# hbell99/DirectVoxGO

Hardware: AMD Instinct MI355X
Metric: train rays/sec (8192-ray batch, 160^3 grid) (higher is better)
Workload: dtype f32

## Files before the change

### directvoxgo_amd/_lib.py

```python
import ctypes
import os
import re

import torch

_HERE = os.path.dirname(os.path.abspath(__file__))
SO_PATH = os.environ.get('DVGO_HIP_SO') or os.path.join(_HERE, 'csrc', 'libdvgo_hip.so')
ABI_VERSION = 11
HEADER_PATH = os.path.join(os.path.dirname(_HERE), 'include', 'dvgo_hip.h')

_lib = None
_nargs = {}


class _Rec2(ctypes.Structure):
    _fields_ = [('step', ctypes.c_int32), ('exp_d', ctypes.c_float), ('alpha', ctypes.c_float), ('T', ctypes.c_float)]


_vp = ctypes.c_void_p
_i64 = ctypes.c_int64
_int = ctypes.c_int
_flt = ctypes.c_float


# ... 87 lines not shown


class _NoCtx:
    def __enter__(self):
        return self

    def __exit__(self, *exc):
        return False


_NOCTX = _NoCtx()


def device_of(t):
    if t.device.index == torch.cuda.current_device():
        return _NOCTX
    return torch.cuda.device_of(t)


_ERR = {-1: 'invalid argument', -2: 'size exceeds 32-bit launch range'}


_profile = None


def profile_start(names):
    global _profile
    _profile = {n: [] for n in names}


def profile_stop():
    global _profile
    prof, _profile = _profile, None
    torch.cuda.synchronize()
    return {n: (len(ev), sum(a.elapsed_time(b) for a, b in ev)) for n, ev in (prof or {}).items()}


def call(name, *args):
    handle = lib()
    if len(args) != _nargs.get(name):
        raise TypeError(f'{name}: {len(args)} arguments given, include/dvgo_hip.h declares {_nargs.get(name, "no such function")}')
    fn = getattr(handle, name)
    if _profile is not None and name in _profile:
        a, b = torch.cuda.Event(enable_timing=True), torch.cuda.Event(enable_timing=True)
        a.record()
        rc = fn(*args)
        b.record()
        _profile[name].append((a, b))
    else:
        rc = fn(*args)
    if rc != 0:
        raise RuntimeError(f'{name} failed: {_ERR.get(rc, "hipError %d" % rc)}')


def f3(x):
    if isinstance(x, torch.Tensor):
        x = x.detach().cpu().tolist()
    return (ctypes.c_float * 3)(*[float(v) for v in x])
```

### directvoxgo_amd/csrc/shade.hip

```cpp
#include "common.h"
#include "x3.h"

#include <type_traits>


static int g_shade_experiment = 0;
static int g_shade_variant = 67;
extern "C" int dvgo_shade_wgrad_x3(const float* G1, const float* gz, const uint64_t* masks, const float* W3, const float* H1,
                                   const float* H2, const float* feat, int C, const float* emb, int E, const int64_t* ray_id,
                                   int64_t M, const int64_t* m_dev, int width, int diffuse, int n_parts, float* part, int form_b,
                                   void* stream);
extern "C" int dvgo_shade_bwd_x3(const float* g_rgb, const float* rgb, const uint64_t* masks, int64_t M, const int64_t* m_dev,
                                 const float* W1, const float* W2, const float* W3, int width, int d_in, int C, int diffuse,
                                 float* g_feat, float* G1, float* gz, void* scratch, int prebuilt, void* stream);

extern "C" int dvgo_shade_fwd_x3(const float* feat, int C, const float* emb, int E, const int64_t* ray_id, int64_t M, const int64_t* m_dev,
                                 const float* W1, const float* b1, const float* W2, const float* b2, const float* W3,
                                 const float* b3, int width, int d_in, int diffuse, float* rgb, float* H1, float* H2,
                                 uint64_t* masks, void* scratch, void* scratch_bwd, int experiment, void* stream);

#define SHADE_THREADS 768
#define SHADE_WAVES (SHADE_THREADS / 64)
#define SHADE_BWD_THREADS 1024
#define SHADE_BWD_WAVES (SHADE_BWD_THREADS / 64)
// ... 977 lines not shown
#pragma unroll
  for (int r = 0; r < 16; ++r) {
    const int i = (r & 3) + 8 * (r >> 2) + 4 * h;
#pragma unroll
    for (int t = 0; t < T; ++t) pW2[(32 * w + i) * WIDTH + 32 * t + j] = aW2[t][r];
    pW1[(32 * w + i) * 64 + j] = aW1[0][r];
    pW1[(32 * w + i) * 64 + 32 + j] = aW1[1][r];
  }
#pragma unroll
  for (int c = 0; c < 3; ++c) {
    const float v = vW3[c] + __shfl_xor(vW3[c], 32);
    if (h == 0) pW3[c * WIDTH + 32 * w + j] = v;
    sgz[c] += __shfl_xor(sgz[c], 32);
  }
  sb1 += __shfl_xor(sb1, 32); sb2 += __shfl_xor(sb2, 32);
  if (h == 0) {
    pb[32 * w + j] = sb1;
    pb[WIDTH + 32 * w + j] = sb2;
    if (j < 8) pb[2 * WIDTH + 8 * w + j] = (w == 0 && j < 3) ? sgz[j] : 0.0f;
    if (T == 2 && j >= 16) pb[2 * WIDTH + 16 * w + j] = 0.0f;
  }
#endif
}
#undef DVGO_OOB

#define SHADE_REDUCE_SLICES 16
__global__ void __launch_bounds__(256)
shade_wgrad_reduce_kernel(const float* __restrict__ part, int n_parts, int n, int W, int d_in, float* __restrict__ out) {
  const int i = blockIdx.x * blockDim.x + threadIdx.x;
  if (i >= n) return;
  int o;
  const int nW2 = W * W, nW1 = W * 64, nW3 = 32 * W;
  if (i < nW2) o = i;
  else if (i < nW2 + nW1) {
    const int r = (i - nW2) >> 6, c = (i - nW2) & 63;
    o = c < d_in ? nW2 + r * d_in + c : -1;
  } else if (i < nW2 + nW1 + nW3) {
    const int e = i - nW2 - nW1;
    o = e < 3 * W ? nW2 + W * d_in + e : -1;
  } else {
    const int e = i - nW2 - nW1 - nW3, base = nW2 + W * d_in + 3 * W;
    if (e < 2 * W) o = base + e;
    else {
      const int c = e - 2 * W;
      o = c < 3 ? base + 2 * W + c : (c >= 8 && c < 11) ? base + 2 * W + c - 8 : -1;
    }
// ... 2 lines not shown
  const int per = (n_parts + SHADE_REDUCE_SLICES - 1) / SHADE_REDUCE_SLICES;
  const int p0 = blockIdx.y * per, p1 = min(n_parts, p0 + per);
  float a0 = 0.0f, a1 = 0.0f, a2 = 0.0f, a3 = 0.0f;
  int p = p0;
  for (; p + 4 <= p1; p += 4) {
    a0 += part[(int64_t)p * n + i];
    a1 += part[(int64_t)(p + 1) * n + i];
    a2 += part[(int64_t)(p + 2) * n + i];
    a3 += part[(int64_t)(p + 3) * n + i];
  }
  for (; p < p1; ++p) a0 += part[(int64_t)p * n + i];
  if (p1 > p0) atomicAdd(out + o, (a0 + a1) + (a2 + a3));
}

extern "C" {

int dvgo_shade_fwd(const float* feat, int C, const float* emb, int E, const int64_t* ray_id, int64_t M, const int64_t* m_dev,
                   const float* W1, const float* b1, const float* W2, const float* b2, const float* W3,
                   const float* b3, int width, int d_in, int diffuse, float* rgb, float* H1, float* H2,
                   uint64_t* masks, void* scratch, void* scratch_bwd, void* stream) {
  if (M < 0 || C <= 0 || E < 0) return DVGO_EINVAL;
  if (M == 0) return 0;
  if (!feat || !emb || !ray_id || !W1 || !b1 || !W2 || !b2 || !W3 || !b3 || !rgb) return DVGO_EINVAL;
  if ((H1 == nullptr) != (H2 == nullptr) || (H1 == nullptr) != (masks == nullptr)) return DVGO_EINVAL;
  const int c_view0 = diffuse ? 3 : 0;
  const int n_view = C - c_view0;
  if (n_view < 0 || d_in != n_view + E) return DVGO_EINVAL;
  if ((width != 128 && width != 64) || d_in > 40) return DVGO_ERANGE;
  if ((g_shade_variant & 1) && scratch != nullptr)
    return dvgo_shade_fwd_x3(feat, C, emb, E, ray_id, M, m_dev, W1, b1, W2, b2, W3, b3, width, d_in, diffuse, rgb, H1, H2, masks,
                             scratch, (g_shade_variant & 2) ? scratch_bwd : nullptr, g_shade_experiment, stream);
  hipStream_t s = (hipStream_t)stream;
  const int64_t n_tiles = (M + 31) / 32;
  const int64_t cap = width == 128 ? 256 : 512;
  int blocks = (int)((n_tiles + SHADE_WAVES - 1) / SHADE_WAVES < cap ? (n_tiles + SHADE_WAVES - 1) / SHADE_WAVES : cap);
#define DVGO_SHADE(W, S1, DIFF)                                                                           \
  shade_fwd_kernel<W, S1, DIFF><<<blocks, SHADE_THREADS, 0, s>>>(feat, C, c_view0, n_view, emb, E, ray_id, M, m_dev, W1, b1, W2, \
                                                          b2, W3, b3, d_in, rgb, H1, H2, (unsigned long long*)masks, g_shade_experiment)
  if (width == 128) {
    if (d_in <= 36) { if (diffuse) DVGO_SHADE(128, 18, true); else DVGO_SHADE(128, 18, false); }
    else            { if (diffuse) DVGO_SHADE(128, 20, true); else DVGO_SHADE(128, 20, false); }
  } else {
    if (d_in <= 12) { if (diffuse) DVGO_SHADE(64, 6, true); else DVGO_SHADE(64, 6, false); }
    else            { if (diffuse) DVGO_SHADE(64, 20, true); else DVGO_SHADE(64, 20, false); }
  }
#undef DVGO_SHADE
  DVGO_LAUNCH_CHECK();
// ... 58 lines not shown
    else if (width == 128)
      shade_wgrad_ring_kernel<128><<<n_parts, 256, 0, (hipStream_t)stream>>>(
          G1, gz, (const unsigned int*)masks, W3, H1, H2, feat, C, c_view0, n_view, emb, E, ray_id, M, m_dev, part, total, tsz);
    else
      shade_wgrad_ring_kernel<64><<<n_parts, 128, 0, (hipStream_t)stream>>>(
          G1, gz, (const unsigned int*)masks, W3, H1, H2, feat, C, c_view0, n_view, emb, E, ray_id, M, m_dev, part, total, tsz);
  } else if (width == 128)
    shade_wgrad_kernel<128><<<n_parts, 256, 0, (hipStream_t)stream>>>(
        G1, gz, (const unsigned int*)masks, W3, H1, H2, feat, C, c_view0, n_view, emb, E, ray_id, M, m_dev, part);
  else
    shade_wgrad_kernel<64><<<n_parts, 128, 0, (hipStream_t)stream>>>(
        G1, gz, (const unsigned int*)masks, W3, H1, H2, feat, C, c_view0, n_view, emb, E, ray_id, M, m_dev, part);
  DVGO_LAUNCH_CHECK();
  const int psize = width * width + width * 64 + 32 * width + 3 * width;
  const int d_in = n_view + E;
  const int tsize = width * width + width * d_in + 3 * width + 2 * width + 3;
  if (!ring && hipMemsetAsync(total, 0, (size_t)tsize * sizeof(float), (hipStream_t)stream) != hipSuccess) return DVGO_EINVAL;
  shade_wgrad_reduce_kernel<<<dim3((psize + 255) / 256, SHADE_REDUCE_SLICES), 256, 0, (hipStream_t)stream>>>(part, n_parts, psize,
                                                                                                       width, d_in, total);
  DVGO_LAUNCH_CHECK();
  return 0;
}

}
```

### directvoxgo_amd/csrc/shade_x3.hip

```cpp
#include "common.h"
#include "x3.h"

#ifndef X3_THREADS
#define X3_THREADS 512
#endif
#define X3_WAVES (X3_THREADS / 64)
#ifndef X3_BWD_THREADS
#define X3_BWD_THREADS 512
#endif
#define X3_BWD_WAVES (X3_BWD_THREADS / 64)
#define X3_STAGE_ROWS 16
#define X3_STAGE_STRIDE 36

__device__ __forceinline__ int x3_acc_feature(int t, int r, int h) { return 32 * t + (r & 3) + 8 * (r >> 2) + 4 * h; }

__device__ __forceinline__ void x3_split1(float v, unsigned short& s0, unsigned short& s1, unsigned short& s2) {
  const unsigned int h = x3_pack(v, 0.f) & 0xffffu;
  const float r = v - __uint_as_float(h << 16);
  const unsigned int m = x3_pack(r, 0.f) & 0xffffu;
  const float q = r - __uint_as_float(m << 16);
  s0 = (unsigned short)h; s1 = (unsigned short)m; s2 = (unsigned short)(x3_pack(q, 0.f) & 0xffffu);
}

template <int WIDTH, int KS1>
// ... 75 lines not shown
  }
  for (int i = tid; i < 2 * T * 16; i += nt) {
    const int tr = i % (T * 16), h = i / (T * 16);
    const int f = x3_acc_feature(tr >> 4, tr & 15, h);
    (&L.b1p[0][0])[i] = b1[f];
    (&L.b2p[0][0])[i] = b2[f];
  }
  if (tid < 4) L.b3[tid] = tid < 3 ? b3[tid] : 0.0f;
}

template <int WIDTH, int KS1, bool DIFFUSE>
__global__ void __launch_bounds__(X3_THREADS)
shade_fwd_x3_kernel(const float* __restrict__ feat, int C, int c_view0, int n_view, const float* __restrict__ emb, int E,
                    const int64_t* __restrict__ ray_id, int64_t M_cap, const int64_t* __restrict__ m_dev,
                    const void* __restrict__ image, float* __restrict__ rgb,
                    float* __restrict__ H1, float* __restrict__ H2, unsigned long long* __restrict__ masks, int experiment) {
  const int64_t M = m_dev ? (*m_dev < M_cap ? *m_dev : M_cap) : M_cap;
  constexpr int T = WIDTH / 32;
  __shared__ __attribute__((aligned(16))) X3Lds<WIDTH, KS1> L;
  x3_copy_image<X3Img<WIDTH, KS1>>(&L, image);
  __syncthreads();
  const int lane = threadIdx.x & 63, h = lane >> 5;
  float* stage = L.stage[threadIdx.x >> 6];
  const bool train = H1 != nullptr;
  const int64_t n_tiles = (M + 31) / 32;
  const int64_t gw = (int64_t)blockIdx.x * (blockDim.x >> 6) + (threadIdx.x >> 6);
  const int64_t nw = (int64_t)gridDim.x * (blockDim.x >> 6);
  const int d_in = n_view + E;
  const int64_t last = M > 0 ? M - 1 : 0;
  auto row_of = [&](int64_t tile) { const int64_t r = tile * 32 + (lane & 31); return r < M ? r : last; };
  float xin[KS1][8];
  auto load_inputs = [&](int64_t tile, int64_t rid) {
    const float* fr = feat + row_of(tile) * C + c_view0;
    const float* er = emb + rid * E - n_view;
#pragma unroll
    for (int s = 0; s < KS1; ++s)
#pragma unroll
      for (int j = 0; j < 8; ++j) {
        const int k = 16 * s + 8 * h + j;
        const int kc = k < d_in ? k : d_in - 1;
        xin[s][j] = *((kc < n_view) ? fr + kc : er + kc);
      }
  };
  int64_t rid_n = 0;
  if (gw < n_tiles) { load_inputs(gw, ray_id[row_of(gw)]); rid_n = ray_id[row_of(gw + nw)]; }
  for (int64_t tile = gw; tile < n_tiles; tile += nw) {
    const int64_t row = tile * 32 + (lane & 31);
// ... 6 lines not shown
#pragma unroll
      for (int j = 0; j < 8; ++j) v[j] = (16 * s + 8 * h + j) < d_in ? xin[s][j] : 0.0f;
      x3_split8(v, x3[s][0], x3[s][1], x3[s][2]);
    }
    load_inputs(tile + nw, rid_n);
    rid_n = ray_id[row_of(tile + 2 * nw)];
    u32x4 h3[2 * T][3];
    unsigned long long mask1 = 0ull;
#pragma unroll
    for (int t = 0; t < T; ++t) {
      f32x16 acc;
#pragma unroll
      for (int r = 0; r < 16; ++r) acc[r] = L.b1p[h][t * 16 + r];
#pragma unroll
      for (int s = 0; s < KS1; ++s)
        x3_mfma6(acc, L.w1s[t][s][0][lane], L.w1s[t][s][1][lane], L.w1s[t][s][2][lane], x3[s][0], x3[s][1], x3[s][2]);
#pragma unroll
      for (int r = 0; r < 16; ++r) acc[r] = dvgo_relu(acc[r]);
      if (train) {
        unsigned int bits = 0u;
#pragma unroll
        for (int r = 0; r < 16; ++r) bits |= dvgo_relu_bit(acc[r]) << r;
        mask1 |= (unsigned long long)bits << (16 * t);
        if (!(experiment & 512)) x3_store_tile(stage, acc, H1 + tile * 32 * WIDTH + 32 * t, WIDTH, lane, rows_valid);
      }
#pragma unroll
      for (int s2 = 0; s2 < 2; ++s2) {
        float v[8];
#pragma unroll
        for (int j = 0; j < 8; ++j) v[j] = acc[8 * s2 + j];
        x3_split8(v, h3[2 * t + s2][0], h3[2 * t + s2][1], h3[2 * t + s2][2]);
      }
      __builtin_amdgcn_sched_barrier(0);
    }
    float p[3] = {0.0f, 0.0f, 0.0f};
    unsigned long long mask2 = 0ull;
#pragma unroll 1
    for (int t2 = 0; t2 < T; ++t2) {
      f32x16 acc2;
#pragma unroll
      for (int r = 0; r < 16; ++r) acc2[r] = L.b2p[h][t2 * 16 + r];
      u32x4 a[2][3];
#pragma unroll
      for (int q = 0; q < 3; ++q) a[0][q] = L.w2s[t2][0][q][lane];
#pragma unroll
      for (int ks = 0; ks < 2 * T; ++ks) {
        if (ks + 1 < 2 * T) {
// ... 892 lines not shown
      float s1 = sb1[t] + red[half][TA * 2 * 16 * 64 + 64 * t + lane];
      s1 += __shfl_xor(s1, 32);
      if (h == 0) pb[T * i + tile] = s1;
    }
  }
#endif
}

extern "C" {

int64_t dvgo_shade_scratch_bytes(int width) {
  if (width == 128) return (int64_t)sizeof(X3Img<128, 3>) > (int64_t)sizeof(X3BwdImg<128>) ? sizeof(X3Img<128, 3>) : sizeof(X3BwdImg<128>);
  if (width == 64) return (int64_t)sizeof(X3Img<64, 3>) > (int64_t)sizeof(X3BwdImg<64>) ? sizeof(X3Img<64, 3>) : sizeof(X3BwdImg<64>);
  return 0;
}

int dvgo_shade_fwd_x3(const float* feat, int C, const float* emb, int E, const int64_t* ray_id, int64_t M, const int64_t* m_dev,
                      const float* W1, const float* b1, const float* W2, const float* b2, const float* W3,
                      const float* b3, int width, int d_in, int diffuse, float* rgb, float* H1, float* H2,
                      uint64_t* masks, void* scratch, void* scratch_bwd, int experiment, void* stream) {
  if (M < 0 || C <= 0 || E < 0) return DVGO_EINVAL;
  if (M == 0) return 0;
  if (!feat || !emb || !ray_id || !W1 || !b1 || !W2 || !b2 || !W3 || !b3 || !rgb || !scratch) return DVGO_EINVAL;
  if ((H1 == nullptr) != (H2 == nullptr) || (H1 == nullptr) != (masks == nullptr)) return DVGO_EINVAL;
  const int c_view0 = diffuse ? 3 : 0;
  const int n_view = C - c_view0;
  if (n_view < 0 || d_in != n_view + E) return DVGO_EINVAL;
  if ((width != 128 && width != 64) || d_in > 48) return DVGO_ERANGE;
  hipStream_t s = (hipStream_t)stream;
  const int64_t n_tiles = (M + 31) / 32;
  const int64_t cap = 256;
  const int blocks = (int)((n_tiles + X3_WAVES - 1) / X3_WAVES < cap ? (n_tiles + X3_WAVES - 1) / X3_WAVES : cap);
#define DVGO_SHADE_X3(W, KS, DIFF)                                                                                       \
  do {                                                                                                                   \
    x3_prep_fwd_kernel<W, KS><<<scratch_bwd ? 64 : 32, 256, 0, s>>>((X3Img<W, KS>*)scratch, (X3BwdImg<W>*)scratch_bwd, W1, b1, W2, b2, W3, b3, d_in); \
    shade_fwd_x3_kernel<W, KS, DIFF><<<blocks, X3_THREADS, 0, s>>>(feat, C, c_view0, n_view, emb, E, ray_id, M, m_dev, scratch, rgb, \
                                                                    H1, H2, (unsigned long long*)masks, experiment);     \
  } while (0)
  if (width == 128) {
    if (diffuse) DVGO_SHADE_X3(128, 3, true); else DVGO_SHADE_X3(128, 3, false);
  } else {
    if (d_in <= 16) { if (diffuse) DVGO_SHADE_X3(64, 1, true); else DVGO_SHADE_X3(64, 1, false); }
    else            { if (diffuse) DVGO_SHADE_X3(64, 3, true); else DVGO_SHADE_X3(64, 3, false); }
  }
#undef DVGO_SHADE_X3
  DVGO_LAUNCH_CHECK();
  return 0;
// ... 63 lines not shown
```

### directvoxgo_amd/shade.py

```python

import torch
import torch.nn as nn

from . import _lib as L
from ._lib import _i64, _int, ptr, stream_of

N_PARTS = 512


class defer_wgrad:
    _active = None
    _streams = {}

    def __init__(self, side_stream=True):
        self.side_stream = side_stream

    def __enter__(self):
        self.pending = []
        defer_wgrad._active = self
        return self

    def __exit__(self, *exc):
        defer_wgrad._active = None
        return False
# ... 56 lines not shown
    gW3 = tot[o:o + 3 * width].view(3, width); o += 3 * width
    gb1, gb2, gb3 = tot[o:o + width], tot[o + width:o + 2 * width], tot[o + 2 * width:o + 2 * width + 3]
    return gW1, gb1, gW2, gb2, gW3, gb3


def _weight_grads(params, wgrad, device, k, n, g_first=None):
    grads = [g_first] + [None] * (n - 1)
    if defer_wgrad._active is not None:
        defer_wgrad._active.submit(params, wgrad, device)
    else:
        grads[k:k + 6] = wgrad()
    return tuple(grads)


class _Shade(torch.autograd.Function):
    @staticmethod
    def forward(ctx, feat, emb, ray_id, W1, b1, W2, b2, W3, b3, diffuse, train, m_dev):
        M, C = feat.shape
        E = emb.shape[1]
        width, d_in = W1.shape
        feat, emb = feat.contiguous(), emb.contiguous()
        train = bool(train) and any(ctx.needs_input_grad)
        rgb = torch.empty((M, 3), dtype=torch.float32, device=feat.device)
        H1 = torch.empty((M, width), dtype=torch.float32, device=feat.device) if train else None
        H2 = torch.empty((M, width), dtype=torch.float32, device=feat.device) if train else None
        masks = torch.empty((M, 4), dtype=torch.int64, device=feat.device) if train else None
        scratch = _scratch(width, feat.device)
        scratch_bwd = _scratch(width, feat.device) if (train and (L.lib().dvgo_shade_variant(-1) & 2)) else None
        with L.device_of(feat):
            L.call('dvgo_shade_fwd', ptr(feat), _int(C), ptr(emb), _int(E), ptr(ray_id), _i64(M), ptr(m_dev), ptr(W1.contiguous()),
                   ptr(b1.contiguous()), ptr(W2.contiguous()), ptr(b2.contiguous()), ptr(W3.contiguous()),
                   ptr(b3.contiguous()), _int(width), _int(d_in), _int(1 if diffuse else 0), ptr(rgb), ptr(H1), ptr(H2),
                   ptr(masks), ptr(scratch), ptr(scratch_bwd), stream_of(feat))
        ctx.scratch_bwd = scratch_bwd if (train and (L.lib().dvgo_shade_variant(-1) & 1)) else None
        if train:
            ctx.save_for_backward(feat, emb, ray_id, W1, W2, W3, rgb, H1, H2, masks)
            ctx.diffuse = diffuse
            ctx.m_dev = m_dev
            ctx.params = (W1, b1, W2, b2, W3, b3)
            ctx.w_versions = (W1._version, W2._version, W3._version)
        return rgb

    @staticmethod
    @torch.autograd.function.once_differentiable
    def backward(ctx, g_rgb):
        feat, emb, ray_id, W1, W2, W3, rgb, H1, H2, masks = ctx.saved_tensors
        diffuse, m_dev = ctx.diffuse, ctx.m_dev
        M, C = feat.shape
        width, d_in = W1.shape
        g_feat = torch.empty_like(feat)
        G1 = torch.empty_like(H1)
        gz = torch.empty_like(rgb)
        prebuilt = ctx.scratch_bwd is not None and W1._version == ctx.w_versions[0] and W2._version == ctx.w_versions[1] \
            and W3._version == ctx.w_versions[2]
        scratch = ctx.scratch_bwd if prebuilt else _scratch(width, feat.device)
        ctx.scratch_bwd = None
        with L.device_of(feat):
            L.call('dvgo_shade_bwd', ptr(g_rgb.contiguous()), ptr(rgb), ptr(masks), _i64(M), ptr(m_dev), ptr(W1.contiguous()),
                   ptr(W2.contiguous()), ptr(W3.contiguous()), _int(width), _int(d_in), _int(C), _int(1 if diffuse else 0),
                   ptr(g_feat), ptr(G1), ptr(gz), ptr(scratch), _int(1 if prebuilt else 0), stream_of(feat))

        def wgrad():
            n_parts = max(1, min(N_PARTS, (M + 255) // 256))
            psize = width * width + width * 64 + 32 * width + 3 * width
            part = torch.empty((n_parts, psize), dtype=torch.float32, device=feat.device)
            tsize = width * width + width * d_in + 5 * width + 3
            tot = torch.empty(tsize, dtype=torch.float32, device=feat.device)
            with L.device_of(feat):
                L.call('dvgo_shade_wgrad', ptr(G1), ptr(gz), ptr(masks), ptr(W3.contiguous()), ptr(H1), ptr(H2), ptr(feat), _int(C), ptr(emb),
                       _int(emb.shape[1]), ptr(ray_id), _i64(M), ptr(m_dev), _int(width), _int(1 if diffuse else 0), _int(n_parts),
                       ptr(part), ptr(tot), stream_of(feat))
            return _unpack_record(tot, width, d_in)

        return _weight_grads(ctx.params, wgrad, feat.device, 3, 12, g_feat if ctx.needs_input_grad[0] else None)


def shade(rgbnet, feat, emb, ray_id, diffuse, m_dev=None):
    layers = head_layers(rgbnet)
    if layers is None or not feat.is_cuda:
        return None
    l1, l2, l3 = layers
    c0 = 3 if diffuse else 0
    if l1.in_features != feat.shape[1] - c0 + emb.shape[1]:
        return None
    return _Shade.apply(feat, emb, ray_id, l1.weight, l1.bias, l2.weight, l2.bias, l3.weight, l3.bias, diffuse,
                        torch.is_grad_enabled(), m_dev)


def posenc_supported(rgbnet, n_freq, emb_dim):
    layers = head_layers_any_din(rgbnet)
    return (layers is not None and layers[0].out_features == 128 and 1 <= n_freq
            and layers[0].in_features == 3 + 6 * n_freq + emb_dim <= 96)


# ... 81 lines not shown
```

### include/dvgo_hip.h

```cpp
#ifndef DVGO_HIP_H
#define DVGO_HIP_H

#include <stdint.h>

#ifdef __cplusplus
extern "C" {
#endif

#define DVGO_EINVAL (-1)
#define DVGO_ERANGE (-2)

#define DVGO_ABI_VERSION 11
int dvgo_abi_version(void);

#define DVGO_TUNE_FEAT_BWD    0
#define DVGO_TUNE_DENSITY_BWD 1
#define DVGO_TUNE_DENSITY_FWD 2
#define DVGO_TUNE_GATHER      3
#define DVGO_TUNE_EXPERIMENT  4
#define DVGO_TUNE_COUNT       8
int dvgo_set_tuning(int key, int value);

int dvgo_infer_t_minmax(const float* rays_o, const float* rays_d,
                        const float* xyz_min, const float* xyz_max,
// ... 168 lines not shown
                          const float* cam_o, int n_cam, float near, float value, void* stream);

int dvgo_shade_fwd(const float* feat, int C, const float* emb, int E, const int64_t* ray_id, int64_t M, const int64_t* m_dev,
                   const float* W1, const float* b1, const float* W2, const float* b2,
                   const float* W3, const float* b3, int width, int d_in, int diffuse,
                   float* rgb, float* H1, float* H2, uint64_t* masks,
                   void* scratch ,
                   void* scratch_bwd ,
                   void* stream);

int64_t dvgo_shade_scratch_bytes(int width);
int dvgo_shade_variant(int flags);

int dvgo_shade_bwd(const float* g_rgb, const float* rgb, const uint64_t* masks, int64_t M, const int64_t* m_dev,
                   const float* W1, const float* W2, const float* W3, int width, int d_in, int C, int diffuse,
                   float* g_feat, float* G1, float* gz, void* scratch,
                   int prebuilt ,
                   void* stream);

int dvgo_shade_wgrad(const float* G1, const float* gz, const uint64_t* masks, const float* W3,
                     const float* H1, const float* H2, const float* feat, int C, const float* emb, int E, const int64_t* ray_id, int64_t M,
                     const int64_t* m_dev, int width, int diffuse, int n_parts, float* part, float* total, void* stream);

int dvgo_march_positions(const float* rays_start, const float* rays_dir, const int64_t* ray_id, const int64_t* step_id,
                         int64_t M, float stepdist, float* pts, void* stream);
int dvgo_shade_pe_fwd(const float* pts, const float* freq, int P, const float* emb, int E, const int64_t* ray_id, int64_t M,
                      const float* W1, const float* b1, const float* W2, const float* b2, const float* W3, const float* b3,
                      int width, int d_in, float* rgb, float* H1, float* H2, uint64_t* masks, void* stream);
int dvgo_shade_pe_bwd(const float* g_rgb, const float* rgb, const uint64_t* masks, int64_t M, const float* W2,
                      const float* W3, int width, float* G1, float* gz, void* stream);
int64_t dvgo_shade_pe_record_size(int width, int d_in);
int dvgo_shade_pe_wgrad(const float* G1, const float* gz, const uint64_t* masks, const float* W3, const float* H1,
                        const float* H2, const float* pts, const float* freq, int P, const float* emb, int E,
                        const int64_t* ray_id, int64_t M, int width, int d_in, int n_parts, float* part, float* total,
                        void* stream);

int dvgo_adam_upd(float* param, const float* grad, float* exp_avg, float* exp_avg_sq,
                  const float* perlr , int64_t n, float step_size,
                  float beta1, float beta2, float eps, int mode, void* stream);

int dvgo_adam_rows(const float* G, int64_t n_vox, int row_stride, int C,
                   float* p_k0, float* m_k0, float* v_k0, float step_size_k0, int mode_k0,
                   float* p_density, float* m_density, float* v_density, float step_size_density, int mode_density,
                   float beta1, float beta2, float eps, void* stream);

int dvgo_total_variation_add_grad(const float* param, float* grad, float wx, float wy, float wz,
// ... 123 lines not shown
```

Baseline: 3.118 million.

## Recompute layer-1 activations in weight-gradient kernel instead of storing H1

```diff
diff --git a/directvoxgo_amd/_lib.py b/directvoxgo_amd/_lib.py
--- a/directvoxgo_amd/_lib.py
+++ b/directvoxgo_amd/_lib.py
@@ -133,6 +133,7 @@
 
 
 _profile = None
+_PROFILE_AS = {'dvgo_shade_wgrad_rebuild': 'dvgo_shade_wgrad'}
 
 
 def profile_start(names):
@@ -152,12 +153,13 @@
     if len(args) != _nargs.get(name):
         raise TypeError(f'{name}: {len(args)} arguments given, include/dvgo_hip.h declares {_nargs.get(name, "no such function")}')
     fn = getattr(handle, name)
-    if _profile is not None and name in _profile:
+    key = _PROFILE_AS.get(name, name)
+    if _profile is not None and key in _profile:
         a, b = torch.cuda.Event(enable_timing=True), torch.cuda.Event(enable_timing=True)
         a.record()
         rc = fn(*args)
         b.record()
-        _profile[name].append((a, b))
+        _profile[key].append((a, b))
     else:
         rc = fn(*args)
     if rc != 0:
diff --git a/directvoxgo_amd/csrc/shade.hip b/directvoxgo_amd/csrc/shade.hip
--- a/directvoxgo_amd/csrc/shade.hip
+++ b/directvoxgo_amd/csrc/shade.hip
@@ -1023,6 +1023,349 @@
   }
 #endif
 }
+template <int WIDTH, int KS1>
+struct ShadeWgradRebuild {
+  static constexpr int NB = 2, NX = 4, NR = 4, TR = 16;
+  float g1[NB][TR][WIDTH], h2[NB][TR][WIDTH];
+  float xf[NX][TR][16];
+  float xe[NX][TR][32];
+  float gz[NB][TR][4];
+  unsigned int m2[NB][TR][4];
+  unsigned int rid[NR][64];
+  u32x4 fb[WIDTH / 32 + 2][3][64];
+  u32x4 xa[KS1][3][64];
+};
+
+template <int WIDTH, int KS1>
+__global__ void __launch_bounds__(2 * WIDTH, 2)
+shade_wgrad_rebuild_kernel(const float* __restrict__ G1, const float* __restrict__ gz, const unsigned int* __restrict__ masks,
+                           const float* __restrict__ W3, const float* __restrict__ W1, const float* __restrict__ b1,
+                           const float* __restrict__ H2, const float* __restrict__ feat, int C, int c_view0, int n_view,
+                           const float* __restrict__ emb, int E, const int64_t* __restrict__ ray_id, int64_t M_cap,
+                           const int64_t* __restrict__ m_dev, float* __restrict__ part, float* __restrict__ total, int total_size) {
+#if defined(__HIP_DEVICE_COMPILE__)
+  for (int i = blockIdx.x * blockDim.x + threadIdx.x; i < total_size; i += gridDim.x * blockDim.x) total[i] = 0.0f;
+  int64_t M;
+  {
+    const int64_t m = m_dev ? (*m_dev < M_cap ? *m_dev : M_cap) : M_cap;
+    M = ((int64_t)__builtin_amdgcn_readfirstlane((int)(m >> 32)) << 32) | (unsigned)__builtin_amdgcn_readfirstlane((int)m);
+  }
+  using Ring = ShadeWgradRebuild<WIDTH, KS1>;
+  constexpr int T = WIDTH / 32, NW = T, NB = Ring::NB, NX = Ring::NX, NR = Ring::NR, TR = Ring::TR;
+  static_assert(T == 4 || T == 2, "widths 128 and 64");
+  static_assert(KS1 == 1 || KS1 == 3, "layer 1 is 1 or 3 k-steps deep");
+  static_assert(sizeof(Ring) <= 80 * 1024, "two workgroups per CU");
+  constexpr int LPR = WIDTH / 4, RPI = 64 / LPR, IPW = TR / RPI / NW;
+  constexpr int DW = NW == 4 ? 2 : NW, FPW = 4 / DW, EPW = 8 / DW;
+  static_assert(IPW == 2 && NB == 2 && TR == 16 && EPW == 4, "double buffer of 16-row tiles: the wait at the top of a tile is vmcnt(0)");
+  __shared__ __attribute__((aligned(16))) Ring L;
+  const int tid = threadIdx.x, lane = tid & 63, h = lane >> 5, j = lane & 31;
+  const int w = __builtin_amdgcn_readfirstlane(tid >> 6);
+  const int dw = NW == 4 ? w - 2 : w;
+  f32x16 aW2[T], aW1[2];
+  float vW3[3] = {0.0f, 0.0f, 0.0f}, sgz[3] = {0.0f, 0.0f, 0.0f};
+#pragma unroll
+  for (int t = 0; t < T; ++t)
+#pragma unroll
+    for (int r = 0; r < 16; ++r) aW2[t][r] = 0.0f;
+#pragma unroll
+  for (int q = 0; q < 2; ++q)
+#pragma unroll
+    for (int r = 0; r < 16; ++r) aW1[q][r] = 0.0f;
+  float sb1 = 0.0f, sb2 = 0.0f;
+  const float w30 = W3[32 * w + j], w31 = W3[WIDTH + 32 * w + j], w32 = W3[2 * WIDTH + 32 * w + j];
+  const int m_idx = 2 * ((j >> 2) & 1) + (w >> 1);
+  const unsigned m_bit = 16 * (w & 1) + (j & 3) + 4 * (j >> 3);
+  const int d_in = n_view + E;
+  const int n_tiles = (int)((M + TR - 1) / TR);
+  auto tile_of = [&](int k) { return (int)blockIdx.x + k * (int)gridDim.x; };
+  u32x4 w1f[KS1][3];
+  {
+    const float* wr = W1 + (32 * w + j) * d_in;
+#pragma unroll
+    for (int s = 0; s < KS1; ++s) {
+      float v[8];
+#pragma unroll
+      for (int e = 0; e < 8; ++e) {
+        const int k = 16 * s + 8 * h + e;
+        const float x = wr[k < d_in ? k : d_in - 1];
+        v[e] = k < d_in ? x : 0.0f;
+      }
+      x3_split8(v, w1f[s][0], w1f[s][1], w1f[s][2]);
+    }
+  }
+  float b1v = b1[32 * w + j];
+#pragma unroll
+  for (int s = 0; s < KS1; ++s)
+    asm volatile("" : "+v"(w1f[s][0]), "+v"(w1f[s][1]), "+v"(w1f[s][2]), "+v"(b1v));
+  const unsigned rows_b = (unsigned)(M * WIDTH * 4);
+  const auto bG1 = __builtin_amdgcn_make_buffer_rsrc((void*)G1, 0, rows_b, 0x00020000);
+  const auto bH2 = __builtin_amdgcn_make_buffer_rsrc((void*)H2, 0, rows_b, 0x00020000);
+  const auto bF = __builtin_amdgcn_make_buffer_rsrc((void*)feat, 0, (unsigned)(M * C * 4), 0x00020000);
+  const auto bE = __builtin_amdgcn_make_buffer_rsrc((void*)emb, 0, DVGO_OOB, 0x00020000);
+  const auto bGz = __builtin_amdgcn_make_buffer_rsrc((void*)gz, 0, (unsigned)(M * 12), 0x00020000);
+  const auto bM = __builtin_amdgcn_make_buffer_rsrc((void*)masks, 0, (unsigned)(M * 32), 0x00020000);
+  const auto bR = __builtin_amdgcn_make_buffer_rsrc((void*)ray_id, 0, (unsigned)(M * 8), 0x00020000);
+  unsigned vo_bulk[IPW], vo_f[FPW], vo_ecol[EPW];
+  int e_row[EPW];
+#pragma unroll
+  for (int i = 0; i < IPW; ++i) vo_bulk[i] = (unsigned)(((IPW * w + i) * RPI + lane / LPR) * WIDTH * 4 + 16 * (lane % LPR));
+#pragma unroll
+  for (int i = 0; i < FPW; ++i) {
+    const int e = 64 * ((dw < 0 ? 0 : dw) + DW * i) + lane, row = e >> 4, col = e & 15;
+    vo_f[i] = col < n_view ? (unsigned)((row * C + c_view0 + col) * 4) : DVGO_OOB;
+  }
+#pragma unroll
+  for (int i = 0; i < EPW; ++i) {
+    const int e = 64 * ((dw < 0 ? 0 : dw) + DW * i) + lane, col = e & 31;
+    e_row[i] = e >> 5;
+    vo_ecol[i] = col < E ? (unsigned)(col * 4) : DVGO_OOB;
+  }
+  const unsigned vo_gz = (lane & 3) < 3 ? (unsigned)(((lane >> 2) * 3 + (lane & 3)) * 4) : DVGO_OOB;
+  const unsigned vo_m2 = (unsigned)(((lane >> 2) * 8 + 4 + (lane & 3)) * 4);
+  const unsigned vo_rid = (unsigned)((lane & (TR - 1)) * 8);
+  auto issue_x = [&](int t) {
+    if (dw < 0) return;
+    const int sx = t & (NX - 1);
+    const unsigned r0 = (unsigned)__builtin_amdgcn_readfirstlane(tile_of(t) * TR);
+#pragma unroll
+    for (int i = 0; i < FPW; ++i)
+      __builtin_amdgcn_raw_ptr_buffer_load_lds(bF, (dvgo_lptr_t)(&L.xf[sx][0][0] + 64 * (dw + DW * i)), 4, vo_f[i], r0 * (unsigned)(C * 4), 0, 0);
+    unsigned rids[EPW];
+#pragma unroll
+    for (int i = 0; i < EPW; ++i) rids[i] = lds_u32<0>(lds_addr(&L.rid[t & (NR - 1)][e_row[i]]));
+    asm volatile("s_waitcnt lgkmcnt(0)" : "+v"(rids[0]), "+v"(rids[1]), "+v"(rids[2]), "+v"(rids[3]));
+#pragma unroll
+    for (int i = 0; i < EPW; ++i)
+      __builtin_amdgcn_raw_ptr_buffer_load_lds(bE, (dvgo_lptr_t)(&L.xe[sx][0][0] + 64 * (dw + DW * i)), 4,
+                                               vo_ecol[i] + rids[i] * (unsigned)(E * 4), 0, 0, 0);
+  };
+  auto issue = [&](int t) {
+    const int sl = t & (NB - 1);
+    const unsigned r0 = (unsigned)__builtin_amdgcn_readfirstlane(tile_of(t) * TR);
+#pragma unroll
+    for (int i = 0; i < IPW; ++i) {
+      const int rl = (IPW * w + i) * RPI;
+      __builtin_amdgcn_raw_ptr_buffer_load_lds(bG1, (dvgo_lptr_t)&L.g1[sl][rl][0], 16, vo_bulk[i], r0 * (WIDTH * 4), 0, 0);
+      __builtin_amdgcn_raw_ptr_buffer_load_lds(bH2, (dvgo_lptr_t)&L.h2[sl][rl][0], 16, vo_bulk[i], r0 * (WIDTH * 4), 0, 0);
+    }
+    if (dw < 0) return;
+    issue_x(t + 2);
+    const unsigned rn = (unsigned)__builtin_amdgcn_readfirstlane(tile_of(t + 3) * TR);
+    if (dw == 0) {
+      __builtin_amdgcn_raw_ptr_buffer_load_lds(bGz, (dvgo_lptr_t)&L.gz[sl][0][0], 4, vo_gz, r0 * 12u, 0, 0);
+      __builtin_amdgcn_raw_ptr_buffer_load_lds(bM, (dvgo_lptr_t)&L.m2[sl][0][0], 4, vo_m2, r0 * 32u, 0, 0);
+    } else {
+      __builtin_amdgcn_raw_ptr_buffer_load_lds(bR, (dvgo_lptr_t)&L.rid[(t + 3) & (NR - 1)][0], 4, vo_rid, rn * 8u, 0, 0);
+    }
+  };
+  const unsigned a_gz = lds_addr(&L.gz[0][8 * h][0]), a_mw = lds_addr(&L.m2[0][8 * h][m_idx]);
+  const unsigned a_g1 = lds_addr(&L.g1[0][8 * h][32 * w + j]), a_h2 = lds_addr(&L.h2[0][8 * h][32 * w + j]);
+  const int xcol = 32 * (w & 1) + j;
+  const bool x_in_f = xcol < n_view, x_ok = xcol < d_in;
+  const unsigned a_x = x_in_f ? lds_addr(&L.xf[0][8 * h][xcol]) : lds_addr(&L.xe[0][8 * h][x_ok ? xcol - n_view : 0]);
+  const unsigned a_fb = lds_addr(&L.fb[0][0][lane]), a_fbw = lds_addr(&L.fb[w][0][lane]), a_xa = lds_addr(&L.xa[0][0][lane]);
+  constexpr unsigned SLOT_ROWS = TR * WIDTH * 4, FB_TILE = 3 * 64 * 16, FB_PIECE = 64 * 16;
+  const int x_row = (j & 3) | (((j >> 3) & 1) << 2) | (((j >> 2) & 1) << 3);
+  const unsigned a_xrf = lds_addr(&L.xf[0][x_row][0]), a_xre = lds_addr(&L.xe[0][x_row][0]) - 4u * (unsigned)n_view;
+  const int xs = NW == 4 ? w - 2 : w;
+  auto build_xa = [&](int k0) {
+    if (xs < 0) return;
+    const unsigned slot = (unsigned)(k0 + (j >> 4)) & (unsigned)(NX - 1);
+    unsigned b_f = a_xrf + slot * (unsigned)(TR * 16 * 4), b_e = a_xre + slot * (unsigned)(TR * 32 * 4);
+    int hh = h;
+    asm volatile("" : "+v"(b_f), "+v"(b_e), "+v"(hh));
+    static_for<0, KS1>([&](auto Sc) {
+      constexpr int s = decltype(Sc)::value;
+      if ((s & 1) != xs) return;
+      float v[8];
+      static_for<0, 8>([&](auto Ec) {
+        constexpr int e = decltype(Ec)::value;
+        const int k = 16 * s + 8 * hh + e, kc = k < d_in ? k : d_in - 1;
+        v[e] = lds_f32<0>((kc < n_view ? b_f : b_e) + 4u * (unsigned)kc);
+      });
+      asm volatile("s_waitcnt lgkmcnt(0)" : "+v"(v[0]), "+v"(v[1]), "+v"(v[2]), "+v"(v[3]), "+v"(v[4]), "+v"(v[5]), "+v"(v[6]), "+v"(v[7]));
+#pragma unroll
+      for (int e = 0; e < 8; ++e) v[e] = (16 * s + 8 * hh + e) < d_in ? v[e] : 0.0f;
+      u32x4 p0, p1, p2;
+      x3_split8(v, p0, p1, p2);
+      lds_store_u32x4<s * FB_TILE>(a_xa, p0);
+      lds_store_u32x4<s * FB_TILE + FB_PIECE>(a_xa, p1);
+      lds_store_u32x4<s * FB_TILE + 2 * FB_PIECE>(a_xa, p2);
+    });
+  };
+  if (tid < 64) {
+#pragma unroll
+    for (int t = 0; t < 3; ++t) {
+      const int64_t row = (int64_t)tile_of(t) * TR + (tid & (TR - 1));
+      L.rid[t][tid] = row < M ? (unsigned int)ray_id[row] : 0u;
+    }
+  }
+  __syncthreads();
+  issue_x(0);
+  issue_x(1);
+  asm volatile("s_waitcnt vmcnt(0)\n\ts_waitcnt lgkmcnt(0)\n\ts_barrier" ::: "memory");
+  build_xa(0);
+  issue(0);
+  u32x4 hf1[3];
+#pragma unroll
+  for (int q = 0; q < 3; ++q) hf1[q] = u32x4{0u, 0u, 0u, 0u};
+  auto body = [&](auto Pc, int k) {
+    constexpr int par = decltype(Pc)::value;
+    asm volatile("s_waitcnt vmcnt(0)\n\ts_waitcnt lgkmcnt(0)\n\ts_barrier" ::: "memory");
+    issue(k + 1);
+    const unsigned b_x = a_x + (unsigned)(k & (NX - 1)) * (x_in_f ? (unsigned)(TR * 16 * 4) : (unsigned)(TR * 32 * 4));
+    u32x4 hf0[3];
+    f32x16 acc;
+    if constexpr (par == 0) {
+      u32x4 xr[KS1][3];
+      static_for<0, KS1 * 3>([&](auto Qc) { constexpr int q = decltype(Qc)::value; xr[q / 3][q % 3] = lds_u32x4<(q / 3) * FB_TILE + (q % 3) * FB_PIECE>(a_xa); });
+      if constexpr (KS1 == 3)
+        asm volatile("s_waitcnt lgkmcnt(0)" : "+v"(xr[0][0]), "+v"(xr[0][1]), "+v"(xr[0][2]), "+v"(xr[1][0]), "+v"(xr[1][1]), "+v"(xr[1][2]),
+                     "+v"(xr[2][0]), "+v"(xr[2][1]), "+v"(xr[2][2]));
+      else
+        asm volatile("s_waitcnt lgkmcnt(0)" : "+v"(xr[0][0]), "+v"(xr[0][1]), "+v"(xr[0][2]));
+#pragma unroll
+      for (int r = 0; r < 16; ++r) acc[r] = b1v;
+#define X3R_MF(A, B) acc = __builtin_amdgcn_mfma_f32_32x32x16_bf16(__builtin_bit_cast(bf16x8, A), __builtin_bit_cast(bf16x8, B), acc, 0, 0, 0)
+#pragma unroll
+      for (int s = 0; s < KS1; ++s) {
+        X3R_MF(xr[s][0], w1f[s][2]); X3R_MF(xr[s][1], w1f[s][1]); X3R_MF(xr[s][2], w1f[s][0]);
+        X3R_MF(xr[s][0], w1f[s][1]); X3R_MF(xr[s][1], w1f[s][0]);
+        X3R_MF(xr[s][0], w1f[s][0]);
+      }
+#undef X3R_MF
+    }
+    if constexpr (par == 0) {
+      float v[8];
+#pragma unroll
+      for (int e = 0; e < 8; ++e) v[e] = dvgo_relu(acc[e]);
+      x3_split8(v, hf0[0], hf0[1], hf0[2]);
+#pragma unroll
+      for (int e = 0; e < 8; ++e) v[e] = dvgo_relu(acc[8 + e]);
+      x3_split8(v, hf1[0], hf1[1], hf1[2]);
+    } else {
+#pragma unroll
+      for (int q = 0; q < 3; ++q) hf0[q] = hf1[q];
+    }
+    lds_store_u32x4<0>(a_fbw, hf0[0]);
+    lds_store_u32x4<FB_PIECE>(a_fbw, hf0[1]);
+    lds_store_u32x4<2 * FB_PIECE>(a_fbw, hf0[2]);
+    u32x4 a2f[3], a1f[3] = {};
+    constexpr int RS = WIDTH * 4 / 256;
+    {
+      float a2[8];
+      static_for<0, 2>([&](auto Hc) {
+        constexpr int e0 = 4 * decltype(Hc)::value;
+        dvgo_f32x4 gq[4];
+        dvgo_f32x2 mp[2], hp[2];
+        static_for<0, 4>([&](auto Ec) {
+          constexpr int e = decltype(Ec)::value;
+          gq[e] = lds_f32x4<16 * (e0 + e) + par * (TR * 16)>(a_gz);
+        });
+        static_for<0, 2>([&](auto Ec) {
+          constexpr int e = 2 * decltype(Ec)::value;
+          mp[e / 2] = lds_f32_pair<4 * (e0 + e) + par * (TR * 4), 4 * (e0 + e + 1) + par * (TR * 4)>(a_mw);
+          hp[e / 2] = lds_f32_pair_st64<(e0 + e) * RS + par * (int)(SLOT_ROWS / 256), (e0 + e + 1) * RS + par * (int)(SLOT_ROWS / 256)>(a_h2);
+        });
+        asm volatile("s_waitcnt lgkmcnt(0)" : "+v"(gq[0]), "+v"(gq[1]), "+v"(gq[2]), "+v"(gq[3]), "+v"(mp[0]), "+v"(mp[1]), "+v"(hp[0]),
+                     "+v"(hp[1]));
+        const unsigned mw[4] = {__float_as_uint(mp[0].x), __float_as_uint(mp[0].y), __float_as_uint(mp[1].x), __float_as_uint(mp[1].y)};
+        const float h2v[4] = {hp[0].x, hp[0].y, hp[1].x, hp[1].y};
+#pragma unroll
+        for (int e = 0; e < 4; ++e) {
+          const float g2v = fmaf(w32, gq[e].z, fmaf(w31, gq[e].y, w30 * gq[e].x));
+          a2[e0 + e] = __uint_as_float(__float_as_uint(g2v) & (unsigned)__builtin_amdgcn_sbfe((int)mw[e], m_bit, 1u));
+          sb2 += a2[e0 + e];
+          vW3[0] = fmaf(gq[e].x, h2v[e], vW3[0]); vW3[1] = fmaf(gq[e].y, h2v[e], vW3[1]); vW3[2] = fmaf(gq[e].z, h2v[e], vW3[2]);
+        }
+        if (w == 0) {
+#pragma unroll
+          for (int e = 0; e < 4; ++e) { sgz[0] += gq[e].x; sgz[1] += gq[e].y; sgz[2] += gq[e].z; }
+        }
+        asm volatile("" : "+v"(a2[e0]), "+v"(a2[e0 + 1]), "+v"(a2[e0 + 2]), "+v"(a2[e0 + 3]), "+v"(sb2), "+v"(vW3[0]), "+v"(vW3[1]), "+v"(vW3[2]));
+      });
+      x3_split8(a2, a2f[0], a2f[1], a2f[2]);
+    }
+    asm volatile("" : "+v"(a2f[0]), "+v"(a2f[1]), "+v"(a2f[2]), "+v"(sb2), "+v"(vW3[0]), "+v"(vW3[1]), "+v"(vW3[2]));
+    if (w < 2) {
+      float xv[8];
+      if (x_in_f) static_for<0, 8>([&](auto Ec) { constexpr int e = decltype(Ec)::value; xv[e] = lds_f32<e * 16 * 4>(b_x); });
+      else static_for<0, 8>([&](auto Ec) { constexpr int e = decltype(Ec)::value; xv[e] = lds_f32<e * 32 * 4>(b_x); });
+      asm volatile("s_waitcnt lgkmcnt(0)" : "+v"(xv[0]), "+v"(xv[1]), "+v"(xv[2]), "+v"(xv[3]), "+v"(xv[4]), "+v"(xv[5]), "+v"(xv[6]), "+v"(xv[7]));
+#pragma unroll
+      for (int e = 0; e < 8; ++e) xv[e] = x_ok ? xv[e] : 0.0f;
+      u32x4 p0, p1, p2;
+      x3_split8(xv, p0, p1, p2);
+      lds_store_u32x4<T * FB_TILE>(a_fbw, p0);
+      lds_store_u32x4<T * FB_TILE + FB_PIECE>(a_fbw, p1);
+      lds_store_u32x4<T * FB_TILE + 2 * FB_PIECE>(a_fbw, p2);
+    }
+    asm volatile("s_waitcnt lgkmcnt(0)\n\ts_barrier" ::: "memory");
+    u32x4 fr[2][3];
+    auto read_tile = [&](auto Pp, u32x4 (&f)[3]) {
+      constexpr int p = decltype(Pp)::value;
+      static_for<0, 3>([&](auto Qc) { constexpr int q = decltype(Qc)::value; f[q] = lds_u32x4<p * FB_TILE + q * FB_PIECE>(a_fb); });
+    };
+    auto wait_tile = [&](u32x4 (&f)[3]) { asm volatile("s_waitcnt lgkmcnt(0)" : "+v"(f[0]), "+v"(f[1]), "+v"(f[2])); };
+    read_tile(std::integral_constant<int, 0>{}, fr[0]);
+    static_for<0, T + 2>([&](auto Pp) {
+      constexpr int p = decltype(Pp)::value;
+      wait_tile(fr[p & 1]);
+      if constexpr (p + 1 < T + 2) read_tile(std::integral_constant<int, p + 1>{}, fr[(p + 1) & 1]);
+      if constexpr (p == T) {
+        dvgo_f32x2 gp[4];
+        static_for<0, 4>([&](auto Ec) {
+          constexpr int e = 2 * decltype(Ec)::value;
+          gp[e / 2] = lds_f32_pair_st64<e * RS + par * (int)(SLOT_ROWS / 256), (e + 1) * RS + par * (int)(SLOT_ROWS / 256)>(a_g1);
+        });
+        asm volatile("s_waitcnt lgkmcnt(0)" : "+v"(gp[0]), "+v"(gp[1]), "+v"(gp[2]), "+v"(gp[3]),
+                     "+v"(fr[(p + 1) & 1][0]), "+v"(fr[(p + 1) & 1][1]), "+v"(fr[(p + 1) & 1][2]));
+        const float g1v[8] = {gp[0].x, gp[0].y, gp[1].x, gp[1].y, gp[2].x, gp[2].y, gp[3].x, gp[3].y};
+#pragma unroll
+        for (int e = 0; e < 8; ++e) sb1 += g1v[e];
+        x3_split8(g1v, a1f[0], a1f[1], a1f[2]);
+      }
+      if constexpr (p < T) x3_mfma6(aW2[p], a2f[0], a2f[1], a2f[2], fr[p & 1][0], fr[p & 1][1], fr[p & 1][2]);
+      else x3_mfma6(aW1[p - T], a1f[0], a1f[1], a1f[2], fr[p & 1][0], fr[p & 1][1], fr[p & 1][2]);
+      __builtin_amdgcn_sched_barrier(0);
+    });
+    if constexpr (par == 1) build_xa(k + 1);
+  };
+  for (int k = 0; tile_of(k) < n_tiles; k += 2) {
+    body(std::integral_constant<int, 0>{}, k);
+    if (tile_of(k + 1) >= n_tiles) break;
+    body(std::integral_constant<int, 1>{}, k + 1);
+  }
+  asm volatile("s_waitcnt vmcnt(0)" ::: "memory");
+  float* p = part + (int64_t)blockIdx.x * (WIDTH * WIDTH + WIDTH * 64 + 32 * WIDTH + 3 * WIDTH);
+  float* pW2 = p;
+  float* pW1 = pW2 + WIDTH * WIDTH;
+  float* pW3 = pW1 + WIDTH * 64;
+  float* pb = pW3 + 32 * WIDTH;
+#pragma unroll
+  for (int r = 0; r < 16; ++r) {
+    const int i = (r & 3) + 8 * (r >> 2) + 4 * h;
+#pragma unroll
+    for (int t = 0; t < T; ++t) pW2[(32 * w + i) * WIDTH + 32 * t + j] = aW2[t][r];
+    pW1[(32 * w + i) * 64 + j] = aW1[0][r];
+    pW1[(32 * w + i) * 64 + 32 + j] = aW1[1][r];
+  }
+#pragma unroll
+  for (int c = 0; c < 3; ++c) {
+    const float v = vW3[c] + __shfl_xor(vW3[c], 32);
+    if (h == 0) pW3[c * WIDTH + 32 * w + j] = v;
+    sgz[c] += __shfl_xor(sgz[c], 32);
+  }
+  sb1 += __shfl_xor(sb1, 32); sb2 += __shfl_xor(sb2, 32);
+  if (h == 0) {
+    pb[32 * w + j] = sb1;
+    pb[WIDTH + 32 * w + j] = sb2;
+    if (j < 8) pb[2 * WIDTH + 8 * w + j] = (w == 0 && j < 3) ? sgz[j] : 0.0f;
+    if (T == 2 && j >= 16) pb[2 * WIDTH + 16 * w + j] = 0.0f;
+  }
+#endif
+}
 #undef DVGO_OOB
 
 #define SHADE_REDUCE_SLICES 16
@@ -1071,7 +1414,8 @@
   if (M < 0 || C <= 0 || E < 0) return DVGO_EINVAL;
   if (M == 0) return 0;
   if (!feat || !emb || !ray_id || !W1 || !b1 || !W2 || !b2 || !W3 || !b3 || !rgb) return DVGO_EINVAL;
-  if ((H1 == nullptr) != (H2 == nullptr) || (H1 == nullptr) != (masks == nullptr)) return DVGO_EINVAL;
+  if ((H2 == nullptr) != (masks == nullptr) || (H1 != nullptr && H2 == nullptr)) return DVGO_EINVAL;
+  if (H1 == nullptr && H2 != nullptr && !((g_shade_variant & 1) && scratch != nullptr)) return DVGO_EINVAL;
   const int c_view0 = diffuse ? 3 : 0;
   const int n_view = C - c_view0;
   if (n_view < 0 || d_in != n_view + E) return DVGO_EINVAL;
@@ -1176,4 +1520,44 @@
   return 0;
 }
 
-}
+static bool shade_rebuild_built(int width, int n_view, int E, int C, int64_t M) {
+  if (n_view > 16 || E > 32 || n_view + E < 1) return false;
+  if (!(width == 128 ? n_view + E <= 40 : n_view + E <= 16)) return false;
+  return M * width * 4 < ((int64_t)1 << 31) && M * C * 4 < ((int64_t)1 << 31);
+}
+
+int dvgo_shade_wgrad_rebuilds(int width, int C, int E, int diffuse, int64_t M) {
+  const int n_view = C - (diffuse ? 3 : 0);
+  if ((g_shade_variant & 195) != 195 || (g_shade_variant & (4 | 8 | 32))) return 0;
+  if ((width != 128 && width != 64) || n_view < 0 || E < 0 || M < 0) return 0;
+  return shade_rebuild_built(width, n_view, E, C, M) ? 1 : 0;
+}
+
+int dvgo_shade_wgrad_rebuild(const float* G1, const float* gz, const uint64_t* masks, const float* W1, const float* b1,
+                             const float* W3, const float* H2, const float* feat, int C, const float* emb, int E,
+                             const int64_t* ray_id, int64_t M, const int64_t* m_dev, int width, int diffuse, int n_parts,
+                             float* part, float* total, void* stream) {
+  if (M < 0 || n_parts <= 0 || C <= 0 || E < 0) return DVGO_EINVAL;
+  if (!G1 || !gz || !masks || !W1 || !b1 || !W3 || !H2 || !feat || !emb || !ray_id || !part || !total) return DVGO_EINVAL;
+  const int c_view0 = diffuse ? 3 : 0;
+  const int n_view = C - c_view0;
+  if (n_view < 0) return DVGO_EINVAL;
+  if ((width != 128 && width != 64) || !shade_rebuild_built(width, n_view, E, C, M)) return DVGO_ERANGE;
+  if (n_parts > 512) n_parts = 512;
+  const int d_in = n_view + E;
+  const int tsize = width * width + width * d_in + 5 * width + 3;
+  if (width == 128)
+    shade_wgrad_rebuild_kernel<128, 3><<<n_parts, 256, 0, (hipStream_t)stream>>>(
+        G1, gz, (const unsigned int*)masks, W3, W1, b1, H2, feat, C, c_view0, n_view, emb, E, ray_id, M, m_dev, part, total, tsize);
+  else
+    shade_wgrad_rebuild_kernel<64, 1><<<n_parts, 128, 0, (hipStream_t)stream>>>(
+        G1, gz, (const unsigned int*)masks, W3, W1, b1, H2, feat, C, c_view0, n_view, emb, E, ray_id, M, m_dev, part, total, tsize);
+  DVGO_LAUNCH_CHECK();
+  const int psize = width * width + width * 64 + 32 * width + 3 * width;
+  shade_wgrad_reduce_kernel<<<dim3((psize + 255) / 256, SHADE_REDUCE_SLICES), 256, 0, (hipStream_t)stream>>>(part, n_parts, psize,
+                                                                                                       width, d_in, total);
+  DVGO_LAUNCH_CHECK();
+  return 0;
+}
+
+}
diff --git a/directvoxgo_amd/csrc/shade_x3.hip b/directvoxgo_amd/csrc/shade_x3.hip
--- a/directvoxgo_amd/csrc/shade_x3.hip
+++ b/directvoxgo_amd/csrc/shade_x3.hip
@@ -121,7 +121,7 @@
   __syncthreads();
   const int lane = threadIdx.x & 63, h = lane >> 5;
   float* stage = L.stage[threadIdx.x >> 6];
-  const bool train = H1 != nullptr;
+  const bool train = masks != nullptr;
   const int64_t n_tiles = (M + 31) / 32;
   const int64_t gw = (int64_t)blockIdx.x * (blockDim.x >> 6) + (threadIdx.x >> 6);
   const int64_t nw = (int64_t)gridDim.x * (blockDim.x >> 6);
@@ -174,7 +174,7 @@
 #pragma unroll
         for (int r = 0; r < 16; ++r) bits |= dvgo_relu_bit(acc[r]) << r;
         mask1 |= (unsigned long long)bits << (16 * t);
-        if (!(experiment & 512)) x3_store_tile(stage, acc, H1 + tile * 32 * WIDTH + 32 * t, WIDTH, lane, rows_valid);
+        if (H1 != nullptr && !(experiment & 512)) x3_store_tile(stage, acc, H1 + tile * 32 * WIDTH + 32 * t, WIDTH, lane, rows_valid);
       }
 #pragma unroll
       for (int s2 = 0; s2 < 2; ++s2) {
@@ -1113,7 +1113,7 @@
   if (M < 0 || C <= 0 || E < 0) return DVGO_EINVAL;
   if (M == 0) return 0;
   if (!feat || !emb || !ray_id || !W1 || !b1 || !W2 || !b2 || !W3 || !b3 || !rgb || !scratch) return DVGO_EINVAL;
-  if ((H1 == nullptr) != (H2 == nullptr) || (H1 == nullptr) != (masks == nullptr)) return DVGO_EINVAL;
+  if ((H2 == nullptr) != (masks == nullptr) || (H1 != nullptr && H2 == nullptr)) return DVGO_EINVAL;
   const int c_view0 = diffuse ? 3 : 0;
   const int n_view = C - c_view0;
   if (n_view < 0 || d_in != n_view + E) return DVGO_EINVAL;
diff --git a/directvoxgo_amd/shade.py b/directvoxgo_amd/shade.py
--- a/directvoxgo_amd/shade.py
+++ b/directvoxgo_amd/shade.py
@@ -102,10 +102,12 @@
         feat, emb = feat.contiguous(), emb.contiguous()
         train = bool(train) and any(ctx.needs_input_grad)
         rgb = torch.empty((M, 3), dtype=torch.float32, device=feat.device)
-        H1 = torch.empty((M, width), dtype=torch.float32, device=feat.device) if train else None
+        scratch = _scratch(width, feat.device)
+        rebuild = bool(train and scratch is not None and L.lib().dvgo_shade_wgrad_rebuilds(
+            _int(width), _int(C), _int(E), _int(1 if diffuse else 0), _i64(M)))
+        H1 = torch.empty((M, width), dtype=torch.float32, device=feat.device) if train and not rebuild else None
         H2 = torch.empty((M, width), dtype=torch.float32, device=feat.device) if train else None
         masks = torch.empty((M, 4), dtype=torch.int64, device=feat.device) if train else None
-        scratch = _scratch(width, feat.device)
         scratch_bwd = _scratch(width, feat.device) if (train and (L.lib().dvgo_shade_variant(-1) & 2)) else None
         with L.device_of(feat):
             L.call('dvgo_shade_fwd', ptr(feat), _int(C), ptr(emb), _int(E), ptr(ray_id), _i64(M), ptr(m_dev), ptr(W1.contiguous()),
@@ -114,7 +116,7 @@
                    ptr(masks), ptr(scratch), ptr(scratch_bwd), stream_of(feat))
         ctx.scratch_bwd = scratch_bwd if (train and (L.lib().dvgo_shade_variant(-1) & 1)) else None
         if train:
-            ctx.save_for_backward(feat, emb, ray_id, W1, W2, W3, rgb, H1, H2, masks)
+            ctx.save_for_backward(feat, emb, ray_id, W1, W2, W3, rgb, H1, H2, masks, b1 if rebuild else None)
             ctx.diffuse = diffuse
             ctx.m_dev = m_dev
             ctx.params = (W1, b1, W2, b2, W3, b3)
@@ -124,12 +126,12 @@
     @staticmethod
     @torch.autograd.function.once_differentiable
     def backward(ctx, g_rgb):
-        feat, emb, ray_id, W1, W2, W3, rgb, H1, H2, masks = ctx.saved_tensors
+        feat, emb, ray_id, W1, W2, W3, rgb, H1, H2, masks, b1 = ctx.saved_tensors
         diffuse, m_dev = ctx.diffuse, ctx.m_dev
         M, C = feat.shape
         width, d_in = W1.shape
         g_feat = torch.empty_like(feat)
-        G1 = torch.empty_like(H1)
+        G1 = torch.empty((masks.shape[0], width), dtype=torch.float32, device=feat.device)
         gz = torch.empty_like(rgb)
         prebuilt = ctx.scratch_bwd is not None and W1._version == ctx.w_versions[0] and W2._version == ctx.w_versions[1] \
             and W3._version == ctx.w_versions[2]
@@ -147,9 +149,14 @@
             tsize = width * width + width * d_in + 5 * width + 3
             tot = torch.empty(tsize, dtype=torch.float32, device=feat.device)
             with L.device_of(feat):
-                L.call('dvgo_shade_wgrad', ptr(G1), ptr(gz), ptr(masks), ptr(W3.contiguous()), ptr(H1), ptr(H2), ptr(feat), _int(C), ptr(emb),
-                       _int(emb.shape[1]), ptr(ray_id), _i64(M), ptr(m_dev), _int(width), _int(1 if diffuse else 0), _int(n_parts),
-                       ptr(part), ptr(tot), stream_of(feat))
+                if H1 is None:
+                    L.call('dvgo_shade_wgrad_rebuild', ptr(G1), ptr(gz), ptr(masks), ptr(W1.contiguous()), ptr(b1.contiguous()),
+                           ptr(W3.contiguous()), ptr(H2), ptr(feat), _int(C), ptr(emb), _int(emb.shape[1]), ptr(ray_id), _i64(M),
+                           ptr(m_dev), _int(width), _int(1 if diffuse else 0), _int(n_parts), ptr(part), ptr(tot), stream_of(feat))
+                else:
+                    L.call('dvgo_shade_wgrad', ptr(G1), ptr(gz), ptr(masks), ptr(W3.contiguous()), ptr(H1), ptr(H2), ptr(feat), _int(C),
+                           ptr(emb), _int(emb.shape[1]), ptr(ray_id), _i64(M), ptr(m_dev), _int(width), _int(1 if diffuse else 0),
+                           _int(n_parts), ptr(part), ptr(tot), stream_of(feat))
             return _unpack_record(tot, width, d_in)
 
         return _weight_grads(ctx.params, wgrad, feat.device, 3, 12, g_feat if ctx.needs_input_grad[0] else None)
diff --git a/include/dvgo_hip.h b/include/dvgo_hip.h
--- a/include/dvgo_hip.h
+++ b/include/dvgo_hip.h
@@ -214,6 +214,12 @@
                      const float* H1, const float* H2, const float* feat, int C, const float* emb, int E, const int64_t* ray_id, int64_t M,
                      const int64_t* m_dev, int width, int diffuse, int n_parts, float* part, float* total, void* stream);
 
+int dvgo_shade_wgrad_rebuild(const float* G1, const float* gz, const uint64_t* masks, const float* W1, const float* b1,
+                             const float* W3, const float* H2, const float* feat, int C, const float* emb, int E,
+                             const int64_t* ray_id, int64_t M, const int64_t* m_dev, int width, int diffuse, int n_parts,
+                             float* part, float* total, void* stream);
+int dvgo_shade_wgrad_rebuilds(int width, int C, int E, int diffuse, int64_t M);
+
 int dvgo_march_positions(const float* rays_start, const float* rays_dir, const int64_t* ray_id, const int64_t* step_id,
                          int64_t M, float stepdist, float* pts, void* stream);
 int dvgo_shade_pe_fwd(const float* pts, const float* freq, int P, const float* emb, int E, const int64_t* ray_id, int64_t M,
```

Measured after the change: 3.097 million. About the same (-0.7%).
